# harryjfowen/PointsToWood

Hardware: AMD Instinct MI355X
Metric: classified points/sec (higher is better)
Workload: dtype f16x3

## Files before the change

### include/p2w.h

```cpp
#ifndef P2W_H
#define P2W_H

#include <stddef.h>
#include <stdint.h>

#ifdef __cplusplus
extern "C" {
#endif

typedef void* p2w_stream_t;

#define P2W_OK 0
#define P2W_EINVAL (-1)
#define P2W_ENULL (-2)
#define P2W_EALIGN (-3)
#define P2W_EWORKSPACE (-4)
#define P2W_EUNSUPPORTED (-5)

#define P2W_MAX_K 64
#define P2W_MAX_K_WIDE 100
#define P2W_MAX_K_CONV 32

int32_t p2w_version(void);
const char* p2w_strerror(int32_t code);
// ... 159 lines not shown
#define P2W_RANGE_LO 0.03125f
#define P2W_RANGE_SLOTS 16
#define P2W_RANGE_WORDS (64 * P2W_RANGE_SLOTS)

void p2w_packed_dims(int32_t N, int32_t K, int32_t* N_pad, int32_t* K_pad);

int32_t p2w_gemm(const float* A, int32_t lda, const float* Wp, int32_t M, int32_t N, int32_t K,
                 const p2w_epilogue* epi, float* out, int32_t ldo, p2w_stream_t stream);

int32_t p2w_sa_conv(const float* P, int32_t ldp, const float* xyzr_src, const int32_t* idx, const int32_t* batch_dst,
                    const float* sf, const int32_t* nbr, const int32_t* deg, int32_t kw, int32_t M,
                    const float* w1r4 , const float* W2p, int32_t C1, int32_t C2,
                    const float* b2, const float* bn_s, const float* bn_t, float* out, int32_t ldo,
                    p2w_stream_t stream);

#define P2W_PREC_F16X3 0
#define P2W_PREC_F16 1
#define P2W_PREC_BF16 2
int32_t p2w_packed_dims_h(int32_t prec, int32_t N, int32_t K, int32_t* N_pad, int32_t* K_pad);

#define P2W_GEMM_TILE_128 1
#define P2W_GEMM_TILE_256 2
#define P2W_GEMM_GENERIC_EPI 4
#define P2W_GEMM_ORDER_ROWS 8
#define P2W_GEMM_ORDER_COLS 16
#define P2W_GEMM_RESIDUAL_H 32
#define P2W_GEMM_STREAMK 64
#define P2W_GEMM_NO_STREAMK 128
#define P2W_GEMM_TILE_64 (1 << 24)
#define P2W_GEMM_NO_TILE_64 (1 << 25)
#define P2W_SA_ITEM_256 1
#define P2W_SA_ITEM_128 2
#define P2W_SA_PACK8 4

int32_t p2w_gemm_h2(int32_t prec, const void* A_h, int32_t ldh_a, const void* Wh, float wscale, int32_t M, int32_t N,
                    int32_t K, const p2w_epilogue* epi, float* out_f32, int32_t ldo, void* out_h, int32_t ldh_o,
                    int32_t flags, p2w_stream_t stream);
size_t p2w_gemm_h2_sk_ws_bytes(void);
int32_t p2w_gemm_h2_sk(int32_t prec, const void* A_h, int32_t ldh_a, const void* Wh, float wscale, int32_t M, int32_t N,
                       int32_t K, const p2w_epilogue* epi, float* out_f32, int32_t ldo, void* out_h, int32_t ldh_o,
                       void* ws, size_t ws_bytes, int32_t flags, p2w_stream_t stream);
size_t p2w_gemm_h2_rowdot_ws_bytes(int32_t M, int32_t N);
int32_t p2w_gemm_h2_rowdot(int32_t prec, const void* A_h, int32_t ldh_a, const void* Wh, float wscale, int32_t M, int32_t N,
                           int32_t K, const p2w_epilogue* epi, const float* dot_w, float dot_b, float* out, void* ws,
                           size_t ws_bytes, int32_t flags, p2w_stream_t stream);
size_t p2w_sa_conv_h_ws_bytes(int32_t M, int32_t flags);
int32_t p2w_sa_conv_h(int32_t prec, const float* P, int32_t ldp, int32_t n_src, const float* xyzr_src, const int32_t* idx,
                      const int32_t* batch_dst, const float* sf, const int32_t* nbr, const int32_t* deg, int32_t kw,
                      int32_t M, const float* w1r4, const void* W2h, float wscale, int32_t C1, int32_t C2,
                      const float* b2, const float* bn_s, const float* bn_t, float* out, int32_t ldo, void* out_h,
                      int32_t ldh, void* ws, size_t ws_bytes, int32_t flags, p2w_stream_t stream);
int32_t p2w_sa_conv_h_rows(int32_t prec, const float* P, int32_t ldp, int32_t n_src, const float* xyzr_src, const int32_t* idx,
                           const int32_t* batch_dst, const float* sf, const int32_t* nbr, const int32_t* deg, int32_t kw,
                           int32_t M, const float* w1r4, const void* W2h, float wscale, int32_t C1, int32_t C2,
                           const float* b2, const float* bn_s, const float* bn_t, float* out, int32_t ldo, void* out_h,
                           int32_t ldh, void* ws, size_t ws_bytes, int32_t flags, const int32_t* src_row, uint32_t* range,
                           p2w_stream_t stream);
int32_t p2w_stem_h2(int32_t prec, const float* xyzr, int32_t n, const float* w, const float* b, int32_t C, float* out,
                    void* out_h, int32_t ldh, uint32_t* range, p2w_stream_t stream);
int32_t p2w_stem_h2_indexed(int32_t prec, const float* xyzr, int32_t n, const float* w, const float* b, int32_t C, float* out,
                            void* out_h, int32_t ldh, uint32_t* range, p2w_stream_t stream);
int32_t p2w_interp_concat_h2(int32_t prec, const float* xc, int32_t Fc, const float* xyzr_c, const float* xyzr_f,
                             const int32_t* nbr, const int32_t* deg, int32_t kw, const float* skip, int32_t Fs, int32_t m,
                             void* out_h, int32_t ldh, p2w_stream_t stream);
int32_t p2w_interp_weights(const float* xyzr_c, const float* xyzr_f, const int32_t* nbr, const int32_t* deg, int32_t kw, int32_t m,
                           void* records, p2w_stream_t stream);
int32_t p2w_concat_xyz_h2(int32_t prec, const float* x, int32_t F, const float* xyzr, int32_t m, void* out_h, int32_t ldh,
                          p2w_stream_t stream);

int32_t p2w_interp_concat(const float* xc, int32_t Fc, const float* xyzr_c, const float* xyzr_f, const int32_t* nbr,
                          const int32_t* deg, int32_t kw, const float* skip, int32_t Fs, int32_t m, float* out,
                          int32_t ldo, p2w_stream_t stream);

int32_t p2w_concat_xyz(const float* x, int32_t F, const float* xyzr, int32_t m, float* out, int32_t ldo,
                       p2w_stream_t stream);

int32_t p2w_segment_max(const float* x, int32_t ldx, int32_t F, const int32_t* ptr, int32_t B, float* out,
                        p2w_stream_t stream);

// ... 59 lines not shown
```

### pointstowood_amd/_lib.py

```python
from __future__ import annotations

import ctypes as C
import os

import torch

_HERE = os.path.dirname(os.path.abspath(__file__))
LIB_PATH = os.path.join(_HERE, "libp2w_gfx950.so")

_vp, _i32, _f32, _sz = C.c_void_p, C.c_int32, C.c_float, C.c_size_t


class Epilogue(C.Structure):
    _fields_ = [("bias", _vp), ("sc0", _vp), ("sh0", _vp), ("sc1", _vp), ("sh1", _vp), ("residual", _vp),
                ("ldr", _i32), ("relu0", _i32), ("relu1", _i32), ("relu2", _i32), ("relu_final", _i32), ("range", _vp),
                ("interp", _vp), ("interp_rows", _i32)]


class BnStage(C.Structure):
    _fields_ = [("dw_w", _vp), ("dw_b", _vp), ("gamma", _vp), ("beta", _vp), ("running_mean", _vp), ("running_var", _vp),
                ("momentum", C.c_double), ("eps", C.c_double), ("relu", _i32)]


SEARCH_X_INDEX_IN_W, SEARCH_Q_ROW_IN_W, SEARCH_BOX = 1, 2, 4
PREC_F16X3, PREC_F16, PREC_BF16 = 0, 1, 2
PREC_OF = {"f16x3": PREC_F16X3, "fp16": PREC_F16, "bf16": PREC_BF16}
GEMM_TILE_128, GEMM_TILE_256, GEMM_GENERIC_EPI, GEMM_ORDER_ROWS, GEMM_ORDER_COLS, GEMM_RESIDUAL_H = 1, 2, 4, 8, 16, 32
GEMM_STREAMK, GEMM_NO_STREAMK = 64, 128
SA_ITEM_256, SA_ITEM_128, SA_PACK8 = 1, 2, 4
CLUSTER_LINK, CLUSTER_COMPRESS, CLUSTER_NUMBER, CLUSTER_ALL = 1, 2, 4, 7
MAX_K_WIDE = 100
EVAL_CHUNK, EVAL_MAX_CLASSES = 4096, 8
LOSS_CHUNK = 4096
EDGE_CHUNK = 1024
BN_GROUP = 16
BN_CHAIN_MAX, BN_CHAIN_ROWS = 3, 32

SIGNATURES = {
    "p2w_version": (_i32, []),
    "p2w_strerror": (C.c_char_p, [_i32]),
    "p2w_pack_xyzr": (_i32, [_vp, _i32, _vp, _vp, _i32, _i32, _vp, _vp, _vp]),
    "p2w_voxel_sample_ws_bytes": (_sz, [_i32]),
    "p2w_voxel_sample": (_i32, [_vp, _vp, _i32, _i32, _f32, _vp, _vp, _vp, _vp, _vp, _vp, _vp, _vp, _vp, _vp, _sz, _vp]),
    "p2w_voxel_sample_table_ws_bytes": (_sz, [_i32, C.c_int64]),
    "p2w_voxel_sample_table": (_i32, [_vp, _vp, _i32, _i32, _f32, _vp, _vp, _vp, _vp, _vp, _vp, _vp, _vp, _vp, _vp, _vp, _vp, C.c_int64,
                                      _vp, _sz, _vp]),
    "p2w_voxel_sample_table_prepare": (_i32, [_vp, _sz, _vp]),
    "p2w_voxel_sample_table_prepared": (_i32, [_vp, _vp, _i32, _i32, _f32, _vp, _vp, _vp, _vp, _vp, _vp, _vp, _vp, _vp, _vp, _vp, _vp, C.c_int64,
                                               _vp, _sz, _vp]),
    "p2w_knn_grid_indexed": (_i32, [_vp, _vp, _vp, _vp, _vp, _vp, _vp, _vp, _i32, _i32, _i32, _vp, _vp, _vp, _i32, _vp]),
    "p2w_ball_query_grid_indexed": (_i32, [_vp, _vp, _vp, _vp, _vp, _vp, _vp, _vp, _i32, _i32, C.c_double, _i32, _vp, _vp, _i32, _vp]),
    "p2w_knn_hint2": (_i32, [_vp, _vp, _vp, _i32, _i32, _vp, _vp, _vp]),
    "p2w_knn_grid": (_i32, [_vp, _vp, _vp, _vp, _vp, _vp, _vp, _i32, _i32, _i32, _vp, _vp, _vp, _i32, _vp]),
    "p2w_ball_query_grid": (_i32, [_vp, _vp, _vp, _vp, _vp, _vp, _vp, _i32, _i32, C.c_double, _i32, _vp, _vp, _i32, _vp]),
    "p2w_index_records": (_i32, [_vp, _vp, _vp, _i32, _i32, _vp, _vp]),
    "p2w_voxel_grid": (_i32, [_vp, _vp, _i32, _i32, _f32, _vp, _vp, _sz, _vp]),
    "p2w_consecutive_cluster": (_i32, [_vp, _i32, _vp, _vp, _vp, _vp, _sz, _vp]),
    "p2w_level_gather": (_i32, [_vp, _vp, _vp, _vp, _i32, _i32, _vp, _vp, _vp]),
    "p2w_ball_query": (_i32, [_vp, _vp, _vp, _vp, _vp, _i32, _i32, C.c_double, _i32, _vp, _vp, _vp, _i32, _vp]),
    "p2w_knn": (_i32, [_vp, _vp, _vp, _vp, _vp, _i32, _i32, _i32, _vp, _vp, _vp, _i32, _vp]),
    "p2w_morton_order_ws_bytes": (_sz, [_i32]),
    "p2w_morton_order": (_i32, [_vp, _i32, _vp, _vp, _vp, _sz, _vp]),
# ... 4 lines not shown
    "p2w_key_runs": (_i32, [_vp, _i32, _i32, _vp, _vp, _vp, _vp, _sz, _vp]),
    "p2w_knn_refine_f64": (_i32, [_vp, _vp, _vp, _vp, _vp, _vp, C.c_double, C.c_double, C.c_double, _vp, _i32, _i32, _i32, _vp, _vp, _vp]),
    "p2w_cell_starts_ws_bytes": (_sz, [C.c_int64]),
    "p2w_cell_starts": (_i32, [_vp, _i32, C.c_int64, _vp, _vp, _sz, _vp]),
    "p2w_vote": (_i32, [_vp, _vp, _i32, _vp, _vp, _i32, _f32, _vp, _vp, _vp]),
    "p2w_euclid_cluster_ws_bytes": (_sz, [C.c_int64]),
    "p2w_euclid_cluster": (_i32, [_vp, _vp, _vp, _vp, _vp, C.c_int64, C.c_double, C.c_int64, C.c_int64, _i32, _vp, _vp, _vp, _vp, _sz, _vp]),
    "p2w_knn_wide_f64": (_i32, [_vp, _vp, _vp, _vp, _vp, C.c_int64, _i32, C.c_double, _vp, _vp]),
    "p2w_pathlen_grow_ws_bytes": (_sz, [C.c_int64]),
    "p2w_pathlen_grow": (_i32, [_vp, _vp, C.c_int64, _i32, _i32, _i32, C.c_double, C.c_double, C.c_double, _vp, _vp, C.c_int64, _vp, _vp,
                                _vp, _sz, _vp]),
    "p2w_pathlen_sssp_ws_bytes": (_sz, [C.c_int64, C.c_int64]),
    "p2w_pathlen_sssp": (_i32, [_vp, _vp, C.c_int64, C.c_int64, _i32, _vp, _vp, _vp, _vp, _sz, _vp]),
    "p2w_pathlen_weights": (_i32, [_vp, _vp, C.c_int64, _vp, _vp]),
    "p2w_confusion_ws_bytes": (_sz, [C.c_int64, _i32, _i32]),
    "p2w_confusion": (_i32, [_vp, _vp, _vp, _vp, C.c_int64, _i32, _i32, _vp, _vp, _vp, _vp, _sz, _vp]),
    "p2w_poly1_focal_ws_bytes": (_sz, [C.c_int64]),
    "p2w_poly1_focal": (_i32, [_vp, _vp, _vp, C.c_int64, C.c_int64, C.c_double, C.c_double, C.c_double, C.c_double, C.c_double, _vp, _vp, _vp,
                               _vp, _sz, _vp]),
    "p2w_tile_bbox": (_i32, [_vp, _vp, _i32, _i32, _vp, _vp]),
    "p2w_tile_bbox_count": (_i32, [_i32, _i32]),
    "p2w_stem": (_i32, [_vp, _i32, _vp, _vp, _i32, _vp, _vp]),
    "p2w_packed_dims": (None, [_i32, _i32, C.POINTER(_i32), C.POINTER(_i32)]),
    "p2w_gemm": (_i32, [_vp, _i32, _vp, _i32, _i32, _i32, C.POINTER(Epilogue), _vp, _i32, _vp]),
    "p2w_sa_conv": (_i32, [_vp, _i32, _vp, _vp, _vp, _vp, _vp, _vp, _i32, _i32, _vp, _vp, _i32, _i32, _vp, _vp, _vp,
                           _vp, _i32, _vp]),
    "p2w_packed_dims_h": (_i32, [_i32, _i32, _i32, C.POINTER(_i32), C.POINTER(_i32)]),
    "p2w_gemm_h2": (_i32, [_i32, _vp, _i32, _vp, _f32, _i32, _i32, _i32, C.POINTER(Epilogue), _vp, _i32, _vp, _i32, _i32, _vp]),
    "p2w_gemm_h2_sk_ws_bytes": (_sz, []),
    "p2w_gemm_h2_sk": (_i32, [_i32, _vp, _i32, _vp, _f32, _i32, _i32, _i32, C.POINTER(Epilogue), _vp, _i32, _vp, _i32, _vp, _sz, _i32, _vp]),
    "p2w_gemm_h2_rowdot_ws_bytes": (_sz, [_i32, _i32]),
    "p2w_gemm_h2_rowdot": (_i32, [_i32, _vp, _i32, _vp, _f32, _i32, _i32, _i32, C.POINTER(Epilogue), _vp, _f32, _vp, _vp, _sz, _i32, _vp]),
    "p2w_sa_conv_h_ws_bytes": (_sz, [_i32, _i32]),
    "p2w_sa_conv_h": (_i32, [_i32, _vp, _i32, _i32, _vp, _vp, _vp, _vp, _vp, _vp, _i32, _i32, _vp, _vp, _f32, _i32, _i32, _vp, _vp,
                             _vp, _vp, _i32, _vp, _i32, _vp, _sz, _i32, _vp]),
    "p2w_stem_h2": (_i32, [_i32, _vp, _i32, _vp, _vp, _i32, _vp, _vp, _i32, _vp, _vp]),
    "p2w_stem_h2_indexed": (_i32, [_i32, _vp, _i32, _vp, _vp, _i32, _vp, _vp, _i32, _vp, _vp]),
    "p2w_sa_conv_h_rows": (_i32, [_i32, _vp, _i32, _i32, _vp, _vp, _vp, _vp, _vp, _vp, _i32, _i32, _vp, _vp, _f32, _i32, _i32, _vp, _vp,
                                  _vp, _vp, _i32, _vp, _i32, _vp, _sz, _i32, _vp, _vp, _vp]),
    "p2w_interp_concat_h2": (_i32, [_i32, _vp, _i32, _vp, _vp, _vp, _vp, _i32, _vp, _i32, _i32, _vp, _i32, _vp]),
    "p2w_interp_weights": (_i32, [_vp, _vp, _vp, _vp, _i32, _i32, _vp, _vp]),
    "p2w_concat_xyz_h2": (_i32, [_i32, _vp, _i32, _vp, _i32, _vp, _i32, _vp]),
    "p2w_interp_concat": (_i32, [_vp, _i32, _vp, _vp, _vp, _vp, _i32, _vp, _i32, _i32, _vp, _i32, _vp]),
    "p2w_concat_xyz": (_i32, [_vp, _i32, _vp, _i32, _vp, _i32, _vp]),
    "p2w_segment_max": (_i32, [_vp, _i32, _i32, _vp, _i32, _vp, _vp]),
    "p2w_rowdot": (_i32, [_vp, _i32, _i32, _vp, _f32, _i32, _vp, _vp]),
    "p2w_fill_batch_nbr": (_i32, [_vp, _i32, _vp, _vp, _vp]),
    "p2w_segment_max_arg": (_i32, [_vp, _i32, _i32, _vp, _i32, _vp, _vp, _vp]),
    "p2w_segment_max_bwd": (_i32, [_vp, _i32, _vp, _vp, _i32, _i32, _vp, _i32, _i32, _vp]),
    "p2w_interp_bwd_ws_bytes": (_sz, [_i32, _i32, _i32]),
    "p2w_interp_bwd": (_i32, [_vp, _i32, _i32, _vp, _vp, _vp, _vp, _i32, _i32, _i32, _vp, _i32, _vp, _sz, _vp]),
    "p2w_edge_l1": (_i32, [_vp, _i32, _vp, _vp, _vp, _vp, _vp, _i32, _i32, _i32, _i32, _vp, _vp, _i32, _vp]),
    "p2w_edge_l1_bwd_ws_bytes": (_sz, [_i32, _i32, _i32]),
    "p2w_edge_l1_bwd": (_i32, [_vp, _i32, _vp, _i32, _vp, _vp, _vp, _i32, _i32, _i32, _vp, _i32, _vp, _vp, _vp, _sz, _vp]),
    "p2w_relu_bn_max_ws_bytes": (_sz, [_i32, _i32, _i32]),
    "p2w_relu_bn_max": (_i32, [_vp, _i32, _vp, _vp, _vp, _vp, _vp, C.c_double, C.c_double, _i32, _i32, _i32, _vp, _vp, _vp, _vp, _vp, _vp, _sz,
                               _vp]),
    "p2w_relu_bn_max_bwd": (_i32, [_vp, _vp, _i32, _vp, _vp, _vp, _vp, _vp, _vp, _i32, _i32, _i32, _vp, _i32, _vp, _vp, _vp, _sz, _vp]),
    "p2w_bn_chain_ws_size": (_sz, [_i32, _i32, _i32]),
    "p2w_bn_chain": (_i32, [_vp, _i32, _vp, _i32, C.POINTER(BnStage), _i32, _i32, _i32, _vp, _i32, _vp, _vp, _vp, _sz, _vp]),
    "p2w_bn_chain_bwd": (_i32, [_vp, _i32, _vp, _i32, _vp, _i32, C.POINTER(BnStage), _i32, _vp, _vp, _i32, _i32, _vp, _i32, _vp, _i32, _vp, _vp,
                                _vp, _vp, _vp, _sz, _vp]),
}

_lib = None

# ... 80 lines not shown
```

### pointstowood_amd/csrc/p2w_feat.hip

```cpp
#include "p2w_hgemm.h"

constexpr int G_BM = 128, G_BN = 128, G_BK = 32, G_LD = 36;

extern "C" void p2w_packed_dims(int32_t N, int32_t K, int32_t* N_pad, int32_t* K_pad) {
    if (N_pad) *N_pad = (N + 255) / 256 * 256;
    if (K_pad) *K_pad = (K + G_BK - 1) / G_BK * G_BK;
}
extern "C" int32_t p2w_packed_dims_h(int32_t prec, int32_t N, int32_t K, int32_t* N_pad, int32_t* K_pad) {
    if (prec < P2W_PREC_F16X3 || prec > P2W_PREC_BF16) return P2W_EINVAL;
    const int ka = prec == P2W_PREC_F16X3 ? 32 : 64;
    if (N_pad) *N_pad = (N + 255) / 256 * 256;
    if (K_pad) *K_pad = (K + ka - 1) / ka * ka;
    return P2W_OK;
}

__device__ __forceinline__ void mma_slab(const float* __restrict__ As, const float* __restrict__ Bs, int wr, int wc, int lane,
                                         f32x16 (&acc)[2][2]) {
    const int r = lane & 31, h = lane >> 5;
#pragma unroll
    for (int kk = 0; kk < G_BK; kk += 8) {
        const float4 a0 = *reinterpret_cast<const float4*>(&As[(wr * 64 + r) * G_LD + kk + 4 * h]);
        const float4 a1 = *reinterpret_cast<const float4*>(&As[(wr * 64 + 32 + r) * G_LD + kk + 4 * h]);
        const float4 b0 = *reinterpret_cast<const float4*>(&Bs[(wc * 64 + r) * G_LD + kk + 4 * h]);
        const float4 b1 = *reinterpret_cast<const float4*>(&Bs[(wc * 64 + 32 + r) * G_LD + kk + 4 * h]);
// ... 432 lines not shown
    part[threadIdx.x] = sum;
    __syncthreads();
    for (int off = 1; off < 1024; off <<= 1) {
        const int v = threadIdx.x >= off ? part[threadIdx.x - off] : 0;
        __syncthreads();
        part[threadIdx.x] += v;
        __syncthreads();
    }
    int run = part[threadIdx.x] - sum;
    for (int b = b0; b < b1; ++b) { const int c = blk_small[b]; blk_small[b] = run; run += c; }
    if (threadIdx.x == 1023) {
        const int ns = part[1023], nl = M - ns;
        counts[0] = ns; counts[1] = nl; counts[2] = (ns + 3) / 4; counts[3] = nl;
    }
}
__global__ __launch_bounds__(SA_PART_BLOCK) void sa_part_scatter_kernel(const int* __restrict__ deg, int kw, int M, const int* __restrict__ blk_small,
                                                                     int* __restrict__ list_small, int* __restrict__ list_large) {
    __shared__ int wsum[SA_PART_BLOCK / 64];
    const int t = blockIdx.x * SA_PART_BLOCK + threadIdx.x, lane = threadIdx.x & 63, wave = threadIdx.x >> 6;
    const bool in = t < M, small = in && min(deg[t], kw) <= 8;
    const unsigned long long bal = __ballot(small);
    const int r_in_wave = __popcll(bal & ((1ull << lane) - 1ull));
    if (lane == 0) wsum[wave] = __popcll(bal);
    __syncthreads();
    int before = 0;
    for (int w = 0; w < wave; ++w) before += wsum[w];
    const int off_s = blk_small[blockIdx.x];
    const int rank_s = before + r_in_wave;
    if (small) list_small[off_s + rank_s] = t;
    else if (in) list_large[(blockIdx.x * SA_PART_BLOCK - off_s) + (threadIdx.x - rank_s)] = t;
}

extern "C" size_t p2w_sa_conv_h_ws_bytes(int32_t M, int32_t flags) { return p2w_ws_bytes([&](P2wArena& a) { sa_conv_carve(a, M < 0 ? 0 : M, flags); }); }

extern "C" int32_t p2w_sa_conv_h_rows(int32_t prec, const float* P, int32_t ldp, int32_t n_src, const float* xyzr_src, const int32_t* idx,
                                 const int32_t* batch_dst, const float* sf, const int32_t* nbr, const int32_t* deg,
                                 int32_t kw, int32_t M, const float* w1r4, const void* W2h, float wscale, int32_t C1,
                                 int32_t C2, const float* b2, const float* bn_s, const float* bn_t, float* out,
                                 int32_t ldo, void* out_h, int32_t ldh, void* ws, size_t ws_bytes, int32_t flags,
                                 const int32_t* src_row, uint32_t* range, p2w_stream_t stream) {
    if (prec < P2W_PREC_F16X3 || prec > P2W_PREC_BF16) return P2W_EINVAL;
    if (M == 0) return P2W_OK;
    P2W_CHECK_PTR(P); P2W_CHECK_PTR(xyzr_src); P2W_CHECK_PTR(idx); P2W_CHECK_PTR(batch_dst); P2W_CHECK_PTR(sf);
    P2W_CHECK_PTR(nbr); P2W_CHECK_PTR(deg); P2W_CHECK_PTR(w1r4); P2W_CHECK_PTR(W2h); P2W_CHECK_PTR(b2);
    P2W_CHECK_PTR(bn_s); P2W_CHECK_PTR(bn_t);
    if (!out && !out_h) return P2W_ENULL;
    P2W_CHECK_ALIGN16(P); P2W_CHECK_ALIGN16(xyzr_src); P2W_CHECK_ALIGN16(w1r4); P2W_CHECK_ALIGN16(W2h);
    if (M < 0 || n_src < 0 || kw <= 0 || kw > 32 || C1 <= 0 || C2 <= 0 || (C1 & 3) || (ldp & 3) || ldp < C1 || (out && ldo < C2) ||
        (out_h && (ldh < C2 || (ldh & 7))) || !(wscale > 0.f))
        return P2W_EINVAL;
    const _Float16* W2 = static_cast<const _Float16*>(W2h);
    if (prec == P2W_PREC_F16X3)
        return launch_sa_conv_h<0>(P, ldp, n_src, xyzr_src, idx, batch_dst, sf, nbr, deg, kw, M, w1r4, W2, wscale, C1, C2, b2, bn_s, bn_t,
                                   out, ldo, static_cast<_Float16*>(out_h), ldh, ws, ws_bytes, flags, p2w_s(stream), src_row, range);
    return p2w_sa_conv_h1_impl(prec, P, ldp, n_src, xyzr_src, idx, batch_dst, sf, nbr, deg, kw, M, w1r4, W2, wscale, C1, C2, b2, bn_s,
                               bn_t, out, ldo, static_cast<_Float16*>(out_h), ldh, ws, ws_bytes, flags, p2w_s(stream), src_row, range);
}

extern "C" int32_t p2w_sa_conv_h(int32_t prec, const float* P, int32_t ldp, int32_t n_src, const float* xyzr_src, const int32_t* idx,
                                 const int32_t* batch_dst, const float* sf, const int32_t* nbr, const int32_t* deg,
                                 int32_t kw, int32_t M, const float* w1r4, const void* W2h, float wscale, int32_t C1,
                                 int32_t C2, const float* b2, const float* bn_s, const float* bn_t, float* out,
                                 int32_t ldo, void* out_h, int32_t ldh, void* ws, size_t ws_bytes, int32_t flags,
                                 p2w_stream_t stream) {
    return p2w_sa_conv_h_rows(prec, P, ldp, n_src, xyzr_src, idx, batch_dst, sf, nbr, deg, kw, M, w1r4, W2h, wscale, C1, C2, b2, bn_s, bn_t,
                              out, ldo, out_h, ldh, ws, ws_bytes, flags, nullptr, nullptr, stream);
// ... 347 lines not shown
```

### pointstowood_amd/csrc/p2w_hgemm.h

```cpp
#pragma once
#include "p2w_common.h"
#include <type_traits>

typedef float f32x16 __attribute__((ext_vector_type(16)));
typedef _Float16 h8 __attribute__((ext_vector_type(8)));
typedef __bf16 bf8 __attribute__((ext_vector_type(8)));
typedef __fp16 hpair __attribute__((ext_vector_type(2)));
typedef _Float16 hpairn __attribute__((ext_vector_type(2)));
typedef __bf16 bpair __attribute__((ext_vector_type(2)));
typedef float fpair __attribute__((ext_vector_type(2)));
typedef __attribute__((address_space(3))) void* lds_vp;
typedef const __attribute__((address_space(1))) void* glb_vp;

constexpr int H_BK = 32;
constexpr int SA_EPI_COLS = 1024;

template <int PREC> struct HCfg {
    static constexpr int planes = PREC == 0 ? 2 : 1;
    static constexpr int kslab = PREC == 0 ? 32 : 64;
    static constexpr int kalign = PREC == 0 ? 32 : 64;
};

template <int PREC>
__device__ __forceinline__ f32x16 h_mfma(h8 a, h8 b, f32x16 c) {
// ... 1066 lines not shown
            asm volatile("" : "+v"(mc.j[u]), "+v"(mc.g[u].x), "+v"(mc.g[u].y), "+v"(mc.g[u].z), "+v"(mc.g[u].w));
        }
#pragma unroll
        for (int i = 0; i < RT; ++i)
#pragma unroll
            for (int q = 0; q < GPT; ++q) asm volatile("" : "+v"(dg_n.d[i][q]));
        __builtin_amdgcn_s_waitcnt(p2w_vmcnt_imm(0));
        if (c0.s == nslab - 1) {
            SaEpiRegs<RT, GPT> e;
#pragma unroll
            for (int j = 0; j < 2; ++j) {
                const int col = min(c0.nt * BN + wc * 64 + j * 32 + (lane & 31), C2 - 1);
                e.bias[j] = Ep[col]; e.s[j] = Ep[SA_EPI_COLS + col]; e.t[j] = Ep[2 * SA_EPI_COLS + col];
            }
#pragma unroll
            for (int i = 0; i < RT; ++i)
#pragma unroll
                for (int q = 0; q < GPT; ++q) e.dsc[i][q] = (c0.mt * (BM / 32) + wr * RT + i >= M) ? -1 : dg_.d[i][q];
            sa_epilogue_regs<PREC, RT, G>(acc, wscale, c0.nt * BN, wc, lane, e, C2, out, ldo, out_h2, ldh, amax);
#pragma unroll
            for (int i = 0; i < RT; ++i)
#pragma unroll
                for (int j = 0; j < 2; ++j)
#pragma unroll
                    for (int e2 = 0; e2 < 16; ++e2) acc[i][j][e2] = 0.f;
        }
        __builtin_amdgcn_sched_barrier(0);
        va = vb; ma = mb; mb = mc; dg_ = dg_n;
        c0 = c1; c1 = c2; c2 = c3; c3 = nxt(c3);
    }
    if (range) range_commit_max(range, amax, lane);
}


__global__ __launch_bounds__(256) void sa_edge_meta_kernel(const float4* __restrict__ xyzr, const int* __restrict__ idx, const int* __restrict__ batch_dst,
                                    const float* __restrict__ sf, const int* __restrict__ nbr, const int* __restrict__ deg, int kw,
                                    int M, int n_src, int ldp4, int G, const int* __restrict__ list, const int* __restrict__ n_list_dev,
                                    const int* __restrict__ src_row, int* __restrict__ meta_j, float4* __restrict__ meta_g, int* __restrict__ desc,
                                    float4* __restrict__ zero_row);
constexpr int SA_PART_BLOCK = 1024;
__global__ __launch_bounds__(SA_PART_BLOCK) void sa_part_count_kernel(const int* __restrict__ deg, int kw, int M, int* __restrict__ blk_small);
__global__ __launch_bounds__(1024) void sa_part_scan_kernel(int* __restrict__ blk_small, int nblk, int M, int* __restrict__ counts);
__global__ __launch_bounds__(SA_PART_BLOCK) void sa_part_scatter_kernel(const int* __restrict__ deg, int kw, int M, const int* __restrict__ blk_small,
                                                                     int* __restrict__ list_small, int* __restrict__ list_large);

struct SaWs {
    float4 *mg_l, *mg_s;
    int *mj_l, *mj_s, *desc_l, *desc_s;
    int *list_s, *list_l, *blk, *counts;
    long t32, t8, nblk;
};
static inline SaWs sa_conv_carve(P2wArena& a, long M, int flags) {
    const bool pack8 = (flags & P2W_SA_PACK8) != 0;
    SaWs W = {};
    W.t32 = M;
    W.t8 = pack8 ? (M + 3) / 4 : 0;
    W.nblk = pack8 ? (M + SA_PART_BLOCK - 1) / SA_PART_BLOCK : 0;
    W.mg_l = a.take<float4>((size_t)W.t32 * 32, 16);
    W.mg_s = a.take<float4>((size_t)W.t8 * 32, 16);
    W.mj_l = a.take<int>((size_t)W.t32 * 32, 4);
    W.mj_s = a.take<int>((size_t)W.t8 * 32, 4);
    W.desc_l = a.take<int>((size_t)W.t32, 4);
    W.desc_s = a.take<int>((size_t)W.t8 * 4, 4);
    if (!pack8) { a.raw(256, 1); return W; }
    W.list_s = a.take<int>((size_t)M, 4);
    W.list_l = a.take<int>((size_t)M, 4);
    W.blk = a.take<int>((size_t)W.nblk, 4);
    W.counts = a.take<int>(16, 4);
    a.raw(1024, 1);
    return W;
}

template <int PREC>
static int32_t launch_sa_conv_h(const float* P, int32_t ldp, int32_t n_src, const float* xyzr_src, const int32_t* idx, const int32_t* batch_dst,
                                const float* sf, const int32_t* nbr, const int32_t* deg, int32_t kw, int32_t M,
                                const float* w1r4, const _Float16* W2h, float wscale, int32_t C1, int32_t C2, const float* b2,
                                const float* bn_s, const float* bn_t, float* out, int32_t ldo, _Float16* out_h2, int32_t ldh,
                                void* ws, size_t ws_bytes, int32_t flags, hipStream_t stream, const int32_t* src_row = nullptr,
                                unsigned* range = nullptr) {
    constexpr int KA = HCfg<PREC>::kalign;
    const int C2pad = (C2 + 255) / 256 * 256, C1pad = (C1 + KA - 1) / KA * KA;
    if (C1pad > 512 || C2 > SA_EPI_COLS || (long)M >= (1L << 25) || ((long)n_src + 1) * (ldp / 4) >= (1L << 31)) return P2W_EUNSUPPORTED;
    if (ldp < C1pad) return P2W_EINVAL;
    P2wArena arena(ws);
    const SaWs L = sa_conv_carve(arena, M, flags);
    if (ws == nullptr || ws_bytes < arena.bytes()) return P2W_EWORKSPACE;
    if (reinterpret_cast<uintptr_t>(ws) & 15u) return P2W_EALIGN;
    const int n_cu = p2w_cu_count();
    const bool wide = (flags & (P2W_SA_ITEM_256 | P2W_SA_ITEM_128)) ? (flags & P2W_SA_ITEM_256) != 0 : C2 > 128;
    const int tpi = wide ? 4 : 8, nNt3 = p2w_cdiv(C2, wide ? 256 : 128);
    const float4* x4 = reinterpret_cast<const float4*>(xyzr_src);
    auto run = [&](auto g_c, const int* list, const int* n_list_dev, const int* tiles_dev, long tiles_max, float4* meta_g, int* meta_j,
                   int* desc) {
        constexpr int G = decltype(g_c)::value;
        const long rows_max = tiles_max * 32;
        sa_edge_meta_kernel<<<p2w_cdiv(rows_max, 256), 256, 0, stream>>>(x4, idx, batch_dst, sf, nbr, deg, kw, M, n_src, ldp / 4, G,
                                                                       list, n_list_dev, src_row, meta_j, meta_g, desc,
                                                                       reinterpret_cast<float4*>(const_cast<float*>(P) + (size_t)n_src * ldp));
        const long items = p2w_cdiv(tiles_max, tpi) * nNt3;
        int grid = (int)(items < n_cu ? items : n_cu);
        if (grid >= 8) grid &= ~7;
        const int nMt3 = (int)p2w_cdiv(tiles_max, tpi);
        if (wide)
            sa_conv16p_kernel<PREC, 256, 2, G><<<grid, 512, 0, stream>>>(
                P, ldp, meta_j, meta_g, desc, tiles_dev, (int)tiles_max, w1r4, C1, C1pad, W2h, (size_t)C2pad * C1pad, wscale, C2, nMt3,
                nNt3, b2, bn_s, bn_t, out, ldo, out_h2, ldh, range);
        else
            sa_conv16p_kernel<PREC, 128, 2, G><<<grid, 512, 0, stream>>>(
                P, ldp, meta_j, meta_g, desc, tiles_dev, (int)tiles_max, w1r4, C1, C1pad, W2h, (size_t)C2pad * C1pad, wscale, C2, nMt3,
                nNt3, b2, bn_s, bn_t, out, ldo, out_h2, ldh, range);
    };
    if (!(flags & P2W_SA_PACK8)) {
        run(std::integral_constant<int, 32>{}, nullptr, nullptr, nullptr, M, L.mg_l, L.mj_l, L.desc_l);
        return P2W_LAUNCH_STATUS();
    }
    int* counts = L.counts;
    sa_part_count_kernel<<<(int)L.nblk, SA_PART_BLOCK, 0, stream>>>(deg, kw, M, L.blk);
    sa_part_scan_kernel<<<1, 1024, 0, stream>>>(L.blk, (int)L.nblk, M, counts);
    sa_part_scatter_kernel<<<(int)L.nblk, SA_PART_BLOCK, 0, stream>>>(deg, kw, M, L.blk, L.list_s, L.list_l);
    run(std::integral_constant<int, 8>{}, L.list_s, counts + 0, counts + 2, L.t8, L.mg_s, L.mj_s, L.desc_s);
    run(std::integral_constant<int, 32>{}, L.list_l, counts + 1, counts + 3, L.t32, L.mg_l, L.mj_l, L.desc_l);
// ... 14 lines not shown
```

### pointstowood_amd/engine.py

```python
from __future__ import annotations

import contextlib
import ctypes as C
import math
from dataclasses import dataclass, field, fields

import torch

from . import _lib
from ._lib import GEMM_RESIDUAL_H, PREC_F16X3, PREC_OF, SA_PACK8, SEARCH_BOX, SEARCH_Q_ROW_IN_W, SEARCH_X_INDEX_IN_W, Epilogue, check, lib, ptr, ws_bytes

BN_EPS = 1e-5
SA_RES = (0.04, 0.08, 0.16)


@dataclass
class Linear:
    w: torch.Tensor
    N: int
    K: int
    bias: torch.Tensor | None = None
    sc0: torch.Tensor | None = None
    sh0: torch.Tensor | None = None
    sc1: torch.Tensor | None = None
# ... 710 lines not shown
        res_h = prec == PREC_F16X3
        Fs = [Cw, 4 * Cw, 8 * Cw, 16 * Cw]
        rows = [N, lv[1].n, lv[2].n, lv[3].n]
        pitch = [pad8(F3 + Fs[f]) for f in range(4)]
        early = geo.early or self._features_early(geo)
        cat = [early["cat0"]] + [newh(rows[f], F3 + Fs[f]) for f in range(1, 4)]
        xh = [hcol(cat[f], F3) for f in range(4)]
        x0 = early["x0"]
        sorted0 = geo.rows0_sorted
        wait = lambda ev: torch.cuda.current_stream().wait_event(ev) if ev is not None else None

        def need(table, key):
            while table.get(key) is None and geo.launch_searches is not None:
                geo.launch_searches(1)
            wait(table.get(key))

        def stage(count):
            if geo.launch_searches is not None and geo.search_stream is not None:
                ev = torch.cuda.Event()
                ev.record()
                geo.launch_searches(count, after=ev)
        if keep is not None:
            keep["stem"] = x0
        x3 = None
        for l in (1, 2, 3):
            p, src, dst = w.sa[l - 1], lv[l - 1], lv[l]
            M, C1, C2, E = dst.n, p["C1"], p["C2"], 4 * p["C2"]
            C1p = pad8(C1)
            P = early["P1"] if l == 1 else self._hoist(xh[l - 1], pitch[l - 1], src.n, p, l)
            need(geo.ev_nbr, l)
            conv = new(M, C2) if (keep is not None or not res_h) else None
            convh = newh(M, C2)
            sa_flags = self.sa_flags | (SA_PACK8 if (l == 1 and self.sa_pack) else 0)
            meta = torch.empty(int(L.p2w_sa_conv_h_ws_bytes(M, sa_flags)) + 65536, dtype=torch.uint8, device=dev)
            if keep is not None:
                keep[f"sa{l}_module.ws"] = meta
            self._call("sa_conv", L.p2w_sa_conv_h_rows, prec, ptr(P), C1p, src.n, ptr(src.xyzr), ptr(dst.idx), ptr(dst.batch),
                       ptr(geo.sf), ptr(dst.nbr), ptr(dst.deg), geo.k, M, ptr(p["w1r4"]), ptr(p["W2"].w16),
                       p["W2"].wscale, C1, C2, ptr(p["b2"]), ptr(p["bn_s"]), ptr(p["bn_t"]), ptr(conv), C2, ptr(convh),
                       pad8(C2), ptr(meta), meta.numel(), sa_flags, ptr(geo.inv0) if (l == 1 and sorted0) else None, self._watch(f"sa{l}", M))
            stage(1 if l < 3 else 2)
            out = new(M, C2) if (keep is not None or l == 3) else None
            def res_chunk(r0, m, bufs):
                e1, e2 = bufs
                self._gemm_h2("gemm_res", convh[r0:], pad8(C2), m, p["g1"], out_h2=e1, ldh_o=pad8(E), watch=f"res{l}.1")
                self._gemm_h2("gemm_res", e1, pad8(E), m, p["g2"], out_h2=e2, ldh_o=pad8(E), watch=f"res{l}.2")
                self._gemm_h2("gemm_res", e2, pad8(E), m, p["g3"], out_h2=e1, ldh_o=pad8(E), watch=f"res{l}.3")
                self._gemm_h2("gemm_res", e1, pad8(E), m, p["g4"], out_f32=None if out is None else out[r0:], ldo=C2,
                              out_h2=xh[l][r0:], ldh_o=pitch[l],
                              residual=convh[r0:] if res_h else conv[r0:], ldr=pad8(C2) if res_h else C2, residual_h=res_h,
                              watch=f"res{l}.4")
            self._chunk_chains(geo, M, E, E // 256, True, lambda rows: (newh(rows, E), newh(rows, E)), res_chunk)
            if l == 3:
                x3 = out
            if keep is not None:
                keep[f"sa{l}_module.conv"], keep[f"sa{l}_module.out"] = conv, out
        M3 = lv[3].n
        cat_g = newh(M3, F3 + 4)
        self._call("concat_xyz", L.p2w_concat_xyz_h2, prec, ptr(x3), F3, ptr(lv[3].xyzr), M3, ptr(cat_g), pad8(F3 + 4))
        h1, h2 = newh(M3, F3), new(M3, F3)
        self._gemm_h2("gemm_mlp", cat_g, pad8(F3 + 4), M3, w.sa4[0], out_h2=h1, ldh_o=pad8(F3), watch="sa4.0")
        self._gemm_h2("gemm_mlp", h1, pad8(F3), M3, w.sa4[1], out_f32=h2, ldo=F3, watch="sa4.1")
        g = new(B, F3)
        self._call("segment_max", L.p2w_segment_max, ptr(h2), F3, F3, ptr(lv[3].ptr), B, ptr(g))
        if keep is not None:
            keep["sa4_module.out"] = g
        nbr4 = torch.empty(M3, dtype=torch.int32, device=dev)
# ... 255 lines not shown
```

Measured before the change: 20.47 million.

## Add resident-weight streaming SA conv kernel for small channel counts

```diff
diff --git a/include/p2w.h b/include/p2w.h
--- a/include/p2w.h
+++ b/include/p2w.h
@@ -215,6 +215,7 @@
 #define P2W_SA_ITEM_256 1
 #define P2W_SA_ITEM_128 2
 #define P2W_SA_PACK8 4
+#define P2W_SA_ITEM_STREAM 8
 
 int32_t p2w_gemm_h2(int32_t prec, const void* A_h, int32_t ldh_a, const void* Wh, float wscale, int32_t M, int32_t N,
                     int32_t K, const p2w_epilogue* epi, float* out_f32, int32_t ldo, void* out_h, int32_t ldh_o,
@@ -228,6 +229,7 @@
                            int32_t K, const p2w_epilogue* epi, const float* dot_w, float dot_b, float* out, void* ws,
                            size_t ws_bytes, int32_t flags, p2w_stream_t stream);
 size_t p2w_sa_conv_h_ws_bytes(int32_t M, int32_t flags);
+size_t p2w_sa_conv_h_ws_need(int32_t M, int32_t C1, int32_t C2, int32_t flags);
 int32_t p2w_sa_conv_h(int32_t prec, const float* P, int32_t ldp, int32_t n_src, const float* xyzr_src, const int32_t* idx,
                       const int32_t* batch_dst, const float* sf, const int32_t* nbr, const int32_t* deg, int32_t kw,
                       int32_t M, const float* w1r4, const void* W2h, float wscale, int32_t C1, int32_t C2,
diff --git a/pointstowood_amd/_lib.py b/pointstowood_amd/_lib.py
--- a/pointstowood_amd/_lib.py
+++ b/pointstowood_amd/_lib.py
@@ -27,7 +27,7 @@
 PREC_OF = {"f16x3": PREC_F16X3, "fp16": PREC_F16, "bf16": PREC_BF16}
 GEMM_TILE_128, GEMM_TILE_256, GEMM_GENERIC_EPI, GEMM_ORDER_ROWS, GEMM_ORDER_COLS, GEMM_RESIDUAL_H = 1, 2, 4, 8, 16, 32
 GEMM_STREAMK, GEMM_NO_STREAMK = 64, 128
-SA_ITEM_256, SA_ITEM_128, SA_PACK8 = 1, 2, 4
+SA_ITEM_256, SA_ITEM_128, SA_PACK8, SA_ITEM_STREAM = 1, 2, 4, 8
 CLUSTER_LINK, CLUSTER_COMPRESS, CLUSTER_NUMBER, CLUSTER_ALL = 1, 2, 4, 7
 MAX_K_WIDE = 100
 EVAL_CHUNK, EVAL_MAX_CLASSES = 4096, 8
@@ -98,6 +98,7 @@
     "p2w_gemm_h2_rowdot_ws_bytes": (_sz, [_i32, _i32]),
     "p2w_gemm_h2_rowdot": (_i32, [_i32, _vp, _i32, _vp, _f32, _i32, _i32, _i32, C.POINTER(Epilogue), _vp, _f32, _vp, _vp, _sz, _i32, _vp]),
     "p2w_sa_conv_h_ws_bytes": (_sz, [_i32, _i32]),
+    "p2w_sa_conv_h_ws_need": (_sz, [_i32, _i32, _i32, _i32]),
     "p2w_sa_conv_h": (_i32, [_i32, _vp, _i32, _i32, _vp, _vp, _vp, _vp, _vp, _vp, _i32, _i32, _vp, _vp, _f32, _i32, _i32, _vp, _vp,
                              _vp, _vp, _i32, _vp, _i32, _vp, _sz, _i32, _vp]),
     "p2w_stem_h2": (_i32, [_i32, _vp, _i32, _vp, _vp, _i32, _vp, _vp, _i32, _vp, _vp]),
diff --git a/pointstowood_amd/csrc/p2w_feat.hip b/pointstowood_amd/csrc/p2w_feat.hip
--- a/pointstowood_amd/csrc/p2w_feat.hip
+++ b/pointstowood_amd/csrc/p2w_feat.hip
@@ -488,6 +488,10 @@
 }
 
 extern "C" size_t p2w_sa_conv_h_ws_bytes(int32_t M, int32_t flags) { return p2w_ws_bytes([&](P2wArena& a) { sa_conv_carve(a, M < 0 ? 0 : M, flags); }); }
+extern "C" size_t p2w_sa_conv_h_ws_need(int32_t M, int32_t C1, int32_t C2, int32_t flags) {
+    if (sa_conv_resident(C1, C2, flags)) return p2w_ws_bytes([&](P2wArena& a) { sa_conv_res_carve(a); });
+    return p2w_sa_conv_h_ws_bytes(M, flags);
+}
 
 extern "C" int32_t p2w_sa_conv_h_rows(int32_t prec, const float* P, int32_t ldp, int32_t n_src, const float* xyzr_src, const int32_t* idx,
                                  const int32_t* batch_dst, const float* sf, const int32_t* nbr, const int32_t* deg,
diff --git a/pointstowood_amd/csrc/p2w_hgemm.h b/pointstowood_amd/csrc/p2w_hgemm.h
--- a/pointstowood_amd/csrc/p2w_hgemm.h
+++ b/pointstowood_amd/csrc/p2w_hgemm.h
@@ -1122,6 +1122,269 @@
     if (range) range_commit_max(range, amax, lane);
 }
 
+constexpr int SAR_CH = 16;
+constexpr int SAR_NB = 4;
+constexpr int SAR_CTRS = 16;
+struct SarChunk {
+    float a[4][SAR_CH];
+    int self[SAR_CH], d[SAR_CH], lst_s[SAR_CH + 4], lst_l[SAR_CH];
+};
+template <int PREC, bool ROWS>
+__global__ __launch_bounds__(256, 2) void sa_conv16r_kernel(const float* __restrict__ P, int ldp4, const float4* __restrict__ xyzr,
+                                                            const int* __restrict__ idx, const int* __restrict__ batch_dst,
+                                                            const float* __restrict__ sf, const int* __restrict__ nbr,
+                                                            const int* __restrict__ deg, int kw, int M,
+                                                            const int* __restrict__ src_row, const float* __restrict__ w1r4,
+                                                            int C1pad, const _Float16* __restrict__ W2h, float wscale, int C2,
+                                                            const float* __restrict__ b2, const float* __restrict__ bn_s,
+                                                            const float* __restrict__ bn_t, float* __restrict__ out, int ldo,
+                                                            _Float16* __restrict__ out_h2, int ldh, unsigned* __restrict__ range,
+                                                            int* __restrict__ ctrs, int nchunks, float4* __restrict__ zero_row) {
+    constexpr int NP = HCfg<PREC>::planes;
+    constexpr int BROW = NP * 128;
+    constexpr int W2_BYTES = 128 * BROW, WR_BYTES = 4 * 64 * 4, EP_BYTES = 3 * 128 * 4;
+    __shared__ __attribute__((aligned(16))) char S[W2_BYTES + WR_BYTES + EP_BYTES + 4 * SAR_NB * sizeof(SarChunk)];
+    float* const Wr = reinterpret_cast<float*>(S + W2_BYTES);
+    float* const Ep = Wr + 4 * 64;
+    const int tid = threadIdx.x, lane = tid & 63, wave = __builtin_amdgcn_readfirstlane(tid >> 6);
+    typedef __attribute__((address_space(3))) SarChunk* sar_lp;
+    const sar_lp CK = (sar_lp)(lds_vp)(S + W2_BYTES + WR_BYTES + EP_BYTES) + SAR_NB * wave;
+    auto bimg = [](int n, int c) { return n * BROW + ((NP == 2 ? (c ^ (n & 15)) : (c ^ ((n >> 1) & 7))) << 4); };
+    {
+        const int cpr = NP * C1pad / 8;
+        for (int i = tid; i < 128 * cpr; i += 256) {
+            const int n = i / cpr, c = i - n * cpr;
+            *reinterpret_cast<uint4*>(S + bimg(n, c)) = *reinterpret_cast<const uint4*>(W2h + (size_t)n * (NP * C1pad) + 8 * c);
+        }
+        for (int i = tid; i < 4 * C1pad; i += 256) Wr[(i / C1pad) * 64 + i % C1pad] = w1r4[i];
+        for (int i = tid; i < C2; i += 256) { Ep[i] = b2[i]; Ep[128 + i] = bn_s[i]; Ep[256 + i] = bn_t[i]; }
+        if (blockIdx.x == 0) for (int i = tid; i < ldp4; i += 256) zero_row[i] = make_float4(0.f, 0.f, 0.f, 0.f);
+    }
+    __syncthreads();
+
+    const int r = lane & 31, h = lane >> 5;
+    int first, stride, limit;
+    if ((gridDim.x & 7) == 0) {
+        const int xcd = blockIdx.x & 7, per = (nchunks + 7) >> 3;
+        first = xcd * per + (blockIdx.x >> 3) * 4 + wave; stride = (gridDim.x >> 3) * 4; limit = min((xcd + 1) * per, nchunks);
+    } else {
+        first = blockIdx.x * 4 + wave; stride = gridDim.x * 4; limit = nchunks;
+    }
+    if (tid == 0 && blockIdx.x == 0) ctrs[0] = nchunks;
+    if (first >= limit) return;
+    const int my_chunks = (limit - first + stride - 1) / stride;
+
+    int nxt_ci = 0, age = 0;
+    bool have_next = false;
+    int n_base = 0, n_ns = 0, n_nt8 = 0, n_nt = 0, n_buf = 0;
+    int s_deg = 0, s_self = 0, s_b = 0;
+    float4 s_pi = make_float4(0.f, 0.f, 0.f, 0.f); float s_s = 1.f;
+    auto setup_l1 = [&]() {
+        const int base = (first + min(nxt_ci, my_chunks - 1) * stride) * SAR_CH;
+        const int ta = min(base + (lane & (SAR_CH - 1)), M - 1);
+        s_deg = deg[ta]; s_self = idx[ta]; s_b = batch_dst[ta];
+    };
+    auto setup_l2 = [&]() { s_pi = xyzr[s_self]; s_s = sf[s_b]; };
+    auto setup_write = [&]() {
+        have_next = nxt_ci < my_chunks;
+        if (!have_next) return;
+        n_base = (first + nxt_ci * stride) * SAR_CH;
+        const bool tv = lane < SAR_CH && n_base + lane < M;
+        const int d = tv ? min(s_deg, kw) : 0;
+        const bool small = tv && d <= 8, large = tv && d > 8;
+        const unsigned long long bs = __ballot(small), bl = __ballot(large), lt = (1ull << lane) - 1ull;
+        n_ns = __popcll(bs); n_nt8 = (n_ns + 3) >> 2; n_nt = n_nt8 + __popcll(bl);
+        n_buf = (n_buf + 1) & (SAR_NB - 1);
+        SarChunk __attribute__((address_space(3)))& c = CK[n_buf];
+        if (lane < SAR_CH) {
+            c.a[0][lane] = s_pi.x / s_s; c.a[1][lane] = s_pi.y / s_s; c.a[2][lane] = s_pi.z / s_s; c.a[3][lane] = s_s;
+            c.self[lane] = s_self; c.d[lane] = d;
+        }
+        if (small) c.lst_s[__popcll(bs & lt)] = lane;
+        if (large) c.lst_l[__popcll(bl & lt)] = lane;
+        __builtin_amdgcn_wave_barrier();
+        ++nxt_ci;
+    };
+
+    struct Tile {
+        int g8;
+        int dsc;
+        int at;
+        bool valid; int jraw, prow; float4 pj;
+    };
+    int c_base = 0, c_ns = 0, c_nt8 = 0, c_nt = 0, c_u = 3, c_buf = 0;
+    bool fin = false;
+    auto stage_n = [&](Tile& T) {
+        if (c_u >= max(c_nt, 3) && !fin) {
+            if (have_next) {
+                c_base = n_base; c_ns = n_ns; c_nt8 = n_nt8; c_nt = n_nt; c_buf = n_buf; c_u = 0;
+                have_next = false; age = 0;
+            } else fin = true;
+        }
+        T.dsc = -1;
+        int li = -1, slot = 0;
+        SarChunk __attribute__((address_space(3)))& c = CK[c_buf];
+        if (fin) T.g8 = -2;
+        else if (c_u >= c_nt) T.g8 = -1;
+        else if (c_u < c_nt8) {
+            T.g8 = 1;
+            const int grp = 4 * c_u + (r >> 3);
+            slot = r & 7;
+            li = grp < c_ns ? c.lst_s[grp] : -1;
+            const int gq = 4 * c_u + (lane & 3);
+            if (gq < c_ns) { const int lq = c.lst_s[gq]; T.dsc = ((c_base + lq) << 6) | c.d[lq]; }
+        } else {
+            T.g8 = 0;
+            li = c.lst_l[c_u - c_nt8];
+            slot = r;
+            if ((lane & 3) == 0) T.dsc = ((c_base + li) << 6) | c.d[li];
+        }
+        const int lc = max(li, 0);
+        T.at = lc | (c_buf << 8);
+        T.valid = li >= 0 && slot < c.d[lc];
+        T.jraw = nbr[T.valid ? (size_t)(c_base + lc) * kw + slot : 0];
+        ++c_u;
+        if (age == 2) setup_write();
+        setup_l2();
+        setup_l1();
+        ++age;
+    };
+    auto stage_x = [&](Tile& T) {
+        const int self = CK[T.at >> 8].self[T.at & 255];
+        int j = T.valid ? T.jraw : self;
+        if (j < 0) j = self;
+        T.pj = xyzr[j];
+        if constexpr (ROWS) T.prow = src_row[j]; else T.prow = j;
+    };
+    struct Feed { float4 g; float4 pv[8]; bool valid; int g8; int dsc; };
+    const float4* const P4 = reinterpret_cast<const float4*>(P);
+    auto stage_g = [&](const Tile& T, Feed& F) {
+        SarChunk __attribute__((address_space(3)))& c = CK[T.at >> 8];
+        const int lc = T.at & 255;
+        const float s = c.a[3][lc], ax = c.a[0][lc], ay = c.a[1][lc], az = c.a[2][lc];
+        float rx = T.pj.x / s - ax, ry = T.pj.y / s - ay, rz = T.pj.z / s - az, rf = T.pj.w;
+        float nrm = sqrtf(((rx * rx) + (ry * ry)) + (rz * rz));
+        if (!T.valid) { rx = 0.f; ry = 0.f; rz = 0.f; rf = 0.f; nrm = 0.f; }
+        float dmax = nrm;
+        if (T.g8 == 0) { dmax = fmaxf(dmax, __shfl_xor(dmax, 16)); dmax = fmaxf(dmax, __shfl_xor(dmax, 8)); }
+        dmax = fmaxf(dmax, __shfl_xor(dmax, 4)); dmax = fmaxf(dmax, __shfl_xor(dmax, 2)); dmax = fmaxf(dmax, __shfl_xor(dmax, 1));
+        const float den = dmax + 1e-8f;
+        F.g = make_float4(rx / den, ry / den, rz / den, rf);
+        F.valid = T.valid; F.g8 = T.g8; F.dsc = T.dsc;
+        const float4* p = P4 + ((unsigned)(T.valid ? T.prow : 0) * (unsigned)ldp4 + 2u * h);
+#pragma unroll
+        for (int s4 = 0; s4 < 4; ++s4) { F.pv[2 * s4] = p[4 * s4]; F.pv[2 * s4 + 1] = p[4 * s4 + 1]; }
+    };
+
+    int offB[4];
+#pragma unroll
+    for (int t = 0; t < 4; ++t) offB[t] = 32 * t + r;
+
+    Tile tb, tc;
+    Feed fa;
+    {
+        setup_l1(); setup_l2(); setup_write(); setup_l1();
+        Tile t0;
+        stage_n(t0); stage_x(t0);
+        stage_n(tb); stage_g(t0, fa);
+        stage_x(tb); stage_n(tc);
+    }
+    float amax = 0.f;
+    while (fa.g8 != -2) {
+        Tile td;
+        stage_n(td);
+        stage_x(tc);
+        Feed fb;
+        stage_g(tb, fb);
+        __builtin_amdgcn_sched_barrier(0);
+        if (fa.g8 < 0) { fa = fb; tb = tc; tc = td; continue; }
+
+        f32x16 acc[2][1][2];
+#pragma unroll
+        for (int wc = 0; wc < 2; ++wc)
+#pragma unroll
+            for (int j = 0; j < 2; ++j)
+#pragma unroll
+                for (int e = 0; e < 16; ++e) acc[wc][0][j][e] = 0.f;
+        const float4 rg = fa.g;
+#pragma unroll
+        for (int s = 0; s < 4; ++s) {
+            if (16 * s >= C1pad) break;
+            const int k = 16 * s + 8 * h;
+            unsigned hiw[4], low[4];
+#pragma unroll
+            for (int half = 0; half < 2; ++half) {
+                const float4 wx = *reinterpret_cast<const float4*>(&Wr[0 * 64 + k + 4 * half]);
+                const float4 wy = *reinterpret_cast<const float4*>(&Wr[1 * 64 + k + 4 * half]);
+                const float4 wz = *reinterpret_cast<const float4*>(&Wr[2 * 64 + k + 4 * half]);
+                const float4 wf = *reinterpret_cast<const float4*>(&Wr[3 * 64 + k + 4 * half]);
+                float4 p = fa.pv[2 * s + half];
+                if (!fa.valid) p = make_float4(0.f, 0.f, 0.f, 0.f);
+                const float gx = rg.x, gy = rg.y, gz = rg.z, gw = rg.w;
+                float v[4];
+                v[0] = fmaxf(fmaf(gw, wf.x, fmaf(gz, wz.x, fmaf(gy, wy.x, fmaf(gx, wx.x, p.x)))), 0.f);
+                v[1] = fmaxf(fmaf(gw, wf.y, fmaf(gz, wz.y, fmaf(gy, wy.y, fmaf(gx, wx.y, p.y)))), 0.f);
+                v[2] = fmaxf(fmaf(gw, wf.z, fmaf(gz, wz.z, fmaf(gy, wy.z, fmaf(gx, wx.z, p.z)))), 0.f);
+                v[3] = fmaxf(fmaf(gw, wf.w, fmaf(gz, wz.w, fmaf(gy, wy.w, fmaf(gx, wx.w, p.w)))), 0.f);
+                if constexpr (PREC == 0) {
+                    unsigned h01, l01, h23, l23;
+                    split_pair(v[0], v[1], h01, l01);
+                    split_pair(v[2], v[3], h23, l23);
+                    hiw[2 * half] = h01; hiw[2 * half + 1] = h23;
+                    low[2 * half] = l01; low[2 * half + 1] = l23;
+                } else {
+                    hiw[2 * half] = pack_pair<PREC>(v[0], v[1]); hiw[2 * half + 1] = pack_pair<PREC>(v[2], v[3]);
+                }
+            }
+            typedef unsigned u32x4 __attribute__((ext_vector_type(4)));
+            const h8 a_hi = __builtin_bit_cast(h8, (u32x4){hiw[0], hiw[1], hiw[2], hiw[3]});
+            h8 a_lo = a_hi;
+            if constexpr (PREC == 0) a_lo = __builtin_bit_cast(h8, (u32x4){low[0], low[1], low[2], low[3]});
+            const int c_hi = NP == 2 ? (s >> 1) * 8 + (s & 1) * 2 + h : 2 * s + h;
+#pragma unroll
+            for (int t = 0; t < 4; ++t) {
+                const h8 b_hi = *reinterpret_cast<const h8*>(S + bimg(offB[t], c_hi));
+                f32x16& a = acc[t >> 1][0][t & 1];
+                if constexpr (PREC == 0) {
+                    const h8 b_lo = *reinterpret_cast<const h8*>(S + bimg(offB[t], c_hi + 4));
+                    a = h_mfma<PREC>(a_lo, b_hi, a);
+                    a = h_mfma<PREC>(a_hi, b_lo, a);
+                }
+                a = h_mfma<PREC>(a_hi, b_hi, a);
+            }
+        }
+        asm volatile("" : "+v"(td.jraw), "+v"(tc.prow), "+v"(tc.pj.x), "+v"(tc.pj.y), "+v"(tc.pj.z), "+v"(tc.pj.w));
+        asm volatile("" : "+v"(s_deg), "+v"(s_self), "+v"(s_b), "+v"(s_s), "+v"(s_pi.x), "+v"(s_pi.y), "+v"(s_pi.z), "+v"(s_pi.w));
+#pragma unroll
+        for (int u = 0; u < 8; ++u) asm volatile("" : "+v"(fb.pv[u].x), "+v"(fb.pv[u].y), "+v"(fb.pv[u].z), "+v"(fb.pv[u].w));
+#pragma unroll
+        for (int wc = 0; wc < 2; ++wc) {
+            float eb[2], es[2], et[2];
+#pragma unroll
+            for (int j = 0; j < 2; ++j) {
+                const int col = min(wc * 64 + j * 32 + r, C2 - 1);
+                eb[j] = Ep[col]; es[j] = Ep[128 + col]; et[j] = Ep[256 + col];
+            }
+            if (fa.g8) {
+                SaEpiRegs<1, 4> e;
+#pragma unroll
+                for (int j = 0; j < 2; ++j) { e.bias[j] = eb[j]; e.s[j] = es[j]; e.t[j] = et[j]; }
+#pragma unroll
+                for (int q = 0; q < 4; ++q) e.dsc[0][q] = __builtin_amdgcn_readlane(fa.dsc, q);
+                sa_epilogue_regs<PREC, 1, 8>(acc[wc], wscale, 0, wc, lane, e, C2, out, ldo, out_h2, ldh, amax);
+            } else {
+                SaEpiRegs<1, 1> e;
+#pragma unroll
+                for (int j = 0; j < 2; ++j) { e.bias[j] = eb[j]; e.s[j] = es[j]; e.t[j] = et[j]; }
+                e.dsc[0][0] = __builtin_amdgcn_readlane(fa.dsc, 0);
+                sa_epilogue_regs<PREC, 1, 32>(acc[wc], wscale, 0, wc, lane, e, C2, out, ldo, out_h2, ldh, amax);
+            }
+        }
+        fa = fb; tb = tc; tc = td;
+    }
+    if (range) range_commit_max(range, amax, lane);
+}
+
 
 __global__ __launch_bounds__(256) void sa_edge_meta_kernel(const float4* __restrict__ xyzr, const int* __restrict__ idx, const int* __restrict__ batch_dst,
                                     const float* __restrict__ sf, const int* __restrict__ nbr, const int* __restrict__ deg, int kw,
@@ -1161,6 +1424,15 @@
     return W;
 }
 
+static inline bool sa_conv_resident(int C1, int C2, int flags) {
+    return C1 <= 64 && C2 <= 128 && !(flags & (P2W_SA_ITEM_STREAM | P2W_SA_ITEM_256 | P2W_SA_ITEM_128));
+}
+static inline int* sa_conv_res_carve(P2wArena& a) {
+    int* ctrs = a.take<int>(SAR_CTRS, 16);
+    a.raw(192, 1);
+    return ctrs;
+}
+
 template <int PREC>
 static int32_t launch_sa_conv_h(const float* P, int32_t ldp, int32_t n_src, const float* xyzr_src, const int32_t* idx, const int32_t* batch_dst,
                                 const float* sf, const int32_t* nbr, const int32_t* deg, int32_t kw, int32_t M,
@@ -1172,11 +1444,28 @@
     const int C2pad = (C2 + 255) / 256 * 256, C1pad = (C1 + KA - 1) / KA * KA;
     if (C1pad > 512 || C2 > SA_EPI_COLS || (long)M >= (1L << 25) || ((long)n_src + 1) * (ldp / 4) >= (1L << 31)) return P2W_EUNSUPPORTED;
     if (ldp < C1pad) return P2W_EINVAL;
+    const int n_cu = p2w_cu_count();
+    if (sa_conv_resident(C1, C2, flags)) {
+        P2wArena arena(ws);
+        int* ctrs = sa_conv_res_carve(arena);
+        if (ws == nullptr || ws_bytes < arena.bytes()) return P2W_EWORKSPACE;
+        if (reinterpret_cast<uintptr_t>(ws) & 15u) return P2W_EALIGN;
+        const int nchunks = p2w_cdiv(M, SAR_CH);
+        int grid = (int)std::min<long>(2L * n_cu, p2w_cdiv(nchunks, 4));
+        if (grid >= 8) grid &= ~7;
+        auto go = [&](auto rows_c) {
+            sa_conv16r_kernel<PREC, decltype(rows_c)::value><<<grid, 256, 0, stream>>>(
+                P, ldp / 4, reinterpret_cast<const float4*>(xyzr_src), idx, batch_dst, sf, nbr, deg, kw, M, src_row, w1r4, C1pad, W2h, wscale,
+                C2, b2, bn_s, bn_t, out, ldo, out_h2, ldh, range, ctrs, nchunks,
+                reinterpret_cast<float4*>(const_cast<float*>(P) + (size_t)n_src * ldp));
+        };
+        if (src_row) go(std::true_type{}); else go(std::false_type{});
+        return P2W_LAUNCH_STATUS();
+    }
     P2wArena arena(ws);
     const SaWs L = sa_conv_carve(arena, M, flags);
     if (ws == nullptr || ws_bytes < arena.bytes()) return P2W_EWORKSPACE;
     if (reinterpret_cast<uintptr_t>(ws) & 15u) return P2W_EALIGN;
-    const int n_cu = p2w_cu_count();
     const bool wide = (flags & (P2W_SA_ITEM_256 | P2W_SA_ITEM_128)) ? (flags & P2W_SA_ITEM_256) != 0 : C2 > 128;
     const int tpi = wide ? 4 : 8, nNt3 = p2w_cdiv(C2, wide ? 256 : 128);
     const float4* x4 = reinterpret_cast<const float4*>(xyzr_src);
diff --git a/pointstowood_amd/engine.py b/pointstowood_amd/engine.py
--- a/pointstowood_amd/engine.py
+++ b/pointstowood_amd/engine.py
@@ -766,7 +766,7 @@
             conv = new(M, C2) if (keep is not None or not res_h) else None
             convh = newh(M, C2)
             sa_flags = self.sa_flags | (SA_PACK8 if (l == 1 and self.sa_pack) else 0)
-            meta = torch.empty(int(L.p2w_sa_conv_h_ws_bytes(M, sa_flags)) + 65536, dtype=torch.uint8, device=dev)
+            meta = torch.empty(int(L.p2w_sa_conv_h_ws_need(M, C1, C2, sa_flags)) + 65536, dtype=torch.uint8, device=dev)
             if keep is not None:
                 keep[f"sa{l}_module.ws"] = meta
             self._call("sa_conv", L.p2w_sa_conv_h_rows, prec, ptr(P), C1p, src.n, ptr(src.xyzr), ptr(dst.idx), ptr(dst.batch),
```

Result: no change. 20.56 million (median of 6 runs) (+0.5%).
